# EPFL-VILAB/omnidata

Measured on AMD Instinct MI355X. Metric: images/sec (384x384) DPT-Hybrid surface-normal inference, higher is better.
Workload: dtype bf16; 1 GPU; DPT-Hybrid-384 normal, batch 32/GPU, bf16, 1xMI355X (BASELINE.json configs[1]); batch_per_gpu=32, global_batch=32, parallelism=replicas x1 (no collective in the loop), ranks_seen=1, inflight=1

## Files before the change

### omnidata_amd/csrc/conv1x1.hip

```cpp
#include "gemm_impl.h"

namespace dptx {

constexpr int C1_STG_PITCH = 144;
constexpr int C1_STG_WAVE = 16 * C1_STG_PITCH;
constexpr int C1_WAVES = 4;

template <int KT, int BN>
constexpr size_t conv1x1_smem_bytes() {
  return (size_t)KT * BN * 128 + (size_t)C1_WAVES * KT * 32 * 128 + (size_t)C1_WAVES * C1_STG_WAVE;
}

template <int DT>
__device__ __forceinline__ void c1_unpack8(const u32x4_t v, float* f) {
#pragma unroll
  for (int i = 0; i < 4; ++i) {
    f[2 * i] = T16<DT>::tof((uint16_t)(v[i] & 0xffffu));
    f[2 * i + 1] = T16<DT>::tof((uint16_t)(v[i] >> 16));
  }
}

template <int DT, int KT, int BN, int FORM>
__global__ __launch_bounds__(64 * C1_WAVES, KT <= 2 ? 2 : 1) void conv1x1_stream_kernel(const GemmParams p) {
#if defined(__HIP_DEVICE_COMPILE__)
  constexpr int NSUB = BN / 64;
  constexpr int KS = KT * 4;
  constexpr int W_BYTES = KT * BN * 128;
  constexpr int A_WAVE = KT * 32 * 128;
  extern __shared__ __attribute__((aligned(16))) char smem[];

  const int tid = threadIdx.x;
  const int lane = tid & 63;
  const int wave = __builtin_amdgcn_readfirstlane(tid >> 6);
  const int lr = lane & 31, lh = lane >> 5;

  const int npan = p.N / BN;
  const int x = (int)blockIdx.x & 7, l = (int)blockIdx.x >> 3;
  const int n0 = (l % npan) * BN;
  const int slots = ((int)gridDim.x / npan) * C1_WAVES;
  const int rb_total = (p.M + 31) >> 5;
  int rb = ((l / npan) * 8 + x) * C1_WAVES + wave;

  const int w_bytes = (int)((long long)p.N * p.ldw * 2);
  const __amdgpu_buffer_rsrc_t rsrcA = __builtin_amdgcn_make_buffer_rsrc(const_cast<void*>(p.A), 0, (int)p.a_bytes, 0x00020000);
  const __amdgpu_buffer_rsrc_t rsrcW = __builtin_amdgcn_make_buffer_rsrc(const_cast<void*>(p.W), 0, w_bytes, 0x00020000);

  char* const sw = smem;
  char* const sa = smem + W_BYTES + wave * A_WAVE;
  char* const stg = smem + W_BYTES + C1_WAVES * A_WAVE + wave * C1_STG_WAVE;

  const int kc = lane & 7, r0 = lane >> 3;
  auto issue_a = [&](int rblk) {
#pragma unroll
    for (int i = 0; i < 4; ++i) {
      const int row = r0 + 8 * i;
      const int m = rblk * 32 + row;
      const bool ok = m < p.M;
      const int mm = ok ? m : 0;
      int rem, ox;
      const int img = row_div(mm, p.a_rpi, p.a_rpi_rcp, false, rem);
      const int oy = row_div(rem, p.Wout, p.wout_rcp, false, ox);
      const int iy = oy * p.stride - p.pad_t, ix = ox * p.stride - p.pad_l;
      const bool valid = ok && ((unsigned)iy < (unsigned)p.Hin) && ((unsigned)ix < (unsigned)p.Win);
      const long long e = (long long)img * p.a_img_stride + p.a_off + ((long long)iy * p.Win + ix) * p.a_pix_stride +
                          (kc ^ ((row >> 1) & 7)) * 8;
      const unsigned base = (unsigned)(e * 2);
#pragma unroll
      for (int kt = 0; kt < KT; ++kt) {
        const unsigned vo = valid ? base + kt * 128 : OOB;
        __builtin_amdgcn_raw_ptr_buffer_load_lds(rsrcA, (__attribute__((address_space(3))) void*)(sa + kt * 4096 + i * 1024), 16, vo,
                                                 0, 0, 0);
      }
    }
  };

  if (rb < rb_total) issue_a(rb);
  for (int idx = wave; idx < KT * (BN / 8); idx += C1_WAVES) {
    const int kt = idx / (BN / 8), rg = idx - kt * (BN / 8);
    const int row = rg * 8 + r0;
    const unsigned vo = (unsigned)(((long long)(n0 + row) * p.ldw + kt * 64 + (kc ^ ((row >> 1) & 7)) * 8) * 2);
    __builtin_amdgcn_raw_ptr_buffer_load_lds(rsrcW, (__attribute__((address_space(3))) void*)(sw + kt * (BN * 128) + rg * 1024), 16, vo,
                                             0, 0, 0);
  }
  float bias_c[NSUB][2];
#pragma unroll
  for (int s = 0; s < NSUB; ++s)
#pragma unroll
    for (int j = 0; j < 2; ++j) bias_c[s][j] = FORM == C1_PLAIN && p.bias != nullptr ? p.bias[n0 + s * 64 + j * 32 + lr] : 0.f;
  asm volatile("s_waitcnt vmcnt(0)" ::: "memory");
  __syncthreads();

  const int swz = (lr >> 1) & 7;
  const unsigned sel = (lr & 1) ? 0x03020706u : 0x05040100u;
  const int cn = lane & 7, rr = lane >> 3;

  const bool has_r = FORM == C1_GN && p.R1 != nullptr;
  const bool r_gn = has_r && p.gn_tab_rgn != 0;

  for (; rb < rb_total; rb += slots) {
    const int m0 = rb * 32;
    float ga[NSUB][8], gd[NSUB][8], gra[NSUB][8], grd[NSUB][8];
    u32x4_t rq[NSUB][4];
    auto load_epi = [&](int s) {
      const int img = m0 / p.gn_hw;
      const float* tab = p.gn_tab + (long long)img * 4 * p.N + n0 + s * 64 + cn * 8;
      if (has_r) {
#pragma unroll
        for (int i = 0; i < 4; ++i) {
          const int m = m0 + 16 * (i >> 1) + rr + 8 * (i & 1);
          rq[s][i] = *(const u32x4_t*)((const uint16_t*)p.R1 + (long long)(p.c_row_off + m) * p.ldc + (n0 + s * 64 + cn * 8));
        }
      }
      *(float4*)&ga[s][0] = *(const float4*)(tab);
      *(float4*)&ga[s][4] = *(const float4*)(tab + 4);
      *(float4*)&gd[s][0] = *(const float4*)(tab + p.N);
      *(float4*)&gd[s][4] = *(const float4*)(tab + p.N + 4);
      if (r_gn) {
        *(float4*)&gra[s][0] = *(const float4*)(tab + 2 * p.N);
        *(float4*)&gra[s][4] = *(const float4*)(tab + 2 * p.N + 4);
        *(float4*)&grd[s][0] = *(const float4*)(tab + 3 * p.N);
        *(float4*)&grd[s][4] = *(const float4*)(tab + 3 * p.N + 4);
      }
    };
    if (FORM == C1_GN) load_epi(0);
    u32x4_t af[KS];
#pragma unroll
    for (int ks = 0; ks < KS; ++ks)
      af[ks] = *(const u32x4_t*)(sa + (ks >> 2) * 4096 + lr * 128 + (((2 * (ks & 3) + lh) ^ swz) << 4));
    asm volatile("s_waitcnt lgkmcnt(0)" ::: "memory");
    const bool prefetch = rb + slots < rb_total;
    if (prefetch) issue_a(rb + slots);

#pragma unroll
    for (int s = 0; s < NSUB; ++s) {
      f32x16_t acc[1][2];
#pragma unroll
      for (int j = 0; j < 2; ++j)
#pragma unroll
        for (int r = 0; r < 16; ++r) acc[0][j][r] = 0.f;
#pragma unroll
      for (int kt = 0; kt < KT; ++kt) {
        u32x4_t bf[4][2];
#pragma unroll
        for (int q = 0; q < 4; ++q)
#pragma unroll
          for (int j = 0; j < 2; ++j)
            bf[q][j] = *(const u32x4_t*)(sw + kt * (BN * 128) + (s * 64 + j * 32 + lr) * 128 + (((2 * q + lh) ^ swz) << 4));
        __builtin_amdgcn_sched_barrier(0);
#pragma unroll
        for (int q = 0; q < 4; ++q)
#pragma unroll
          for (int j = 0; j < 2; ++j) acc[0][j] = T16<DT>::mfma32(af[kt * 4 + q], bf[q][j], acc[0][j]);
      }
      if (s == 0) {
        __builtin_amdgcn_sched_barrier(0);
        asm volatile("s_waitcnt vmcnt(0)" ::: "memory");
      }
      if (FORM == C1_STATS || (FORM == C1_PLAIN && p.gn_part != nullptr)) gn_records<1, 2>(p, m0, n0 + s * 64, 0, 0, lr, lh, acc);
      if (FORM == C1_STATS) continue;
      if (FORM == C1_GN && s + 1 < NSUB) load_epi(s + 1);

#pragma unroll
      for (int h = 0; h < 2; ++h) {
        asm volatile("" ::: "memory");
        __builtin_amdgcn_wave_barrier();
#pragma unroll
        for (int j = 0; j < 2; ++j)
#pragma unroll
          for (int t = 0; t < 4; ++t) {
            float v0 = acc[0][j][8 * h + 2 * t] + bias_c[s][j], v1 = acc[0][j][8 * h + 2 * t + 1] + bias_c[s][j];
            if (FORM != C1_GN && p.act == 1) { v0 = fmaxf(v0, 0.f); v1 = fmaxf(v1, 0.f); }
            const uint32_t own = T16<DT>::pack2(v0, v1);
            const uint32_t nb = (uint32_t)__builtin_amdgcn_update_dpp(0, (int)own, 0xB1, 0xf, 0xf, false);
            const uint32_t o = __builtin_amdgcn_perm(nb, own, sel);
            const int rl = ((2 * t) & 3) + (lr & 1) + 8 * (t >> 1) + 4 * lh;
            *(uint32_t*)(stg + rl * C1_STG_PITCH + (j * 32 + (lr & ~1)) * 2) = o;
          }
        asm volatile("" ::: "memory");
        __builtin_amdgcn_wave_barrier();
#pragma unroll
        for (int pp = 0; pp < 2; ++pp) {
          const int rl = rr + 8 * pp;
          u32x4_t d = *(const u32x4_t*)(stg + rl * C1_STG_PITCH + cn * 16);
          const int m = m0 + 16 * h + rl;
          if (FORM == C1_GN) {
            float f[8];
            c1_unpack8<DT>(d, f);
#pragma unroll
            for (int e = 0; e < 8; ++e) f[e] = __builtin_fmaf(f[e], ga[s][e], gd[s][e]);
            if (has_r) {
              float r[8];
              c1_unpack8<DT>(rq[s][2 * h + pp], r);
              if (r_gn) {
#pragma unroll
                for (int e = 0; e < 8; ++e) r[e] = __builtin_fmaf(r[e], gra[s][e], grd[s][e]);
              }
#pragma unroll
              for (int e = 0; e < 8; ++e) f[e] = __fadd_rn(f[e], r[e]);
            }
            if (p.act == 1) {
#pragma unroll
              for (int e = 0; e < 8; ++e) f[e] = fmaxf(f[e], 0.f);
            }
#pragma unroll
            for (int e = 0; e < 4; ++e) d[e] = T16<DT>::pack2(f[2 * e], f[2 * e + 1]);
          }
          if (FORM == C1_GN || m < p.M) *(u32x4_t*)((uint16_t*)p.C + (long long)(p.c_row_off + m) * p.ldc + (n0 + s * 64 + cn * 8)) = d;
        }
      }
    }
  }
#endif
}

bool conv1x1_stream_eligible(int mode, const GemmParams& p) {
  if (mode != MODE_BF16 && mode != MODE_FP16) return false;
  if (p.ksz != 1 || p.pad_t != 0 || p.pad_l != 0 || (p.stride != 1 && p.stride != 2)) return false;
  if (p.K != p.Cin || (p.K != 64 && p.K != 128 && p.K != 256) || p.N % 64 != 0) return false;
  if (p.a_fp32 || p.c_fp32 || p.epi2 || p.a_relu || p.R1 != nullptr || p.R2 != nullptr || p.bias_per_img) return false;
  if (p.c_rpi != 0x7fffffff || p.C8 != nullptr || p.C16 != nullptr || p.out_scale != 0.f) return false;
  if (p.row_stats != nullptr || p.ln_stats != nullptr || (p.act != 0 && p.act != 1)) return false;
  if (p.ldc % 8 != 0 || p.a_pix_stride % 8 != 0 || p.a_off % 8 != 0 || p.a_img_stride % 8 != 0) return false;
  if (p.a_bytes <= 0 || p.a_bytes >= (1ll << 31) || (long long)p.N * p.ldw * 2 >= (1ll << 31) || p.M >= (1 << 23)) return false;
  return true;
}

bool conv1x1_stream_adopted(const GemmParams& p) {
  if (p.stride != 1) return false;
  if (p.K == 64) return p.N == 256 || p.N == 64;
  if (p.K == 128) return p.N == 512;
  if (p.K == 256) return p.N == 64 || p.N == 128 || (p.N == 256 && p.a_rpi >= 48 * 48);
  return false;
}

bool conv1x1_gn_eligible(int mode, const GemmParams& p) {
  if (!conv1x1_stream_eligible(mode, p) || p.stride != 1 || p.bias != nullptr || p.act != 0) return false;
  const int cpg = p.N / 32;
  if (p.a_rpi % 32 != 0 || p.M % p.a_rpi != 0 || p.N > 1024 || (cpg & (cpg - 1)) != 0) return false;
  return p.c_row_off == 0 && p.ldc == p.N;
}

bool conv1x1_gn_adopted(const GemmParams& p) {
  if (p.K == 64) return p.N == 256;
  if (p.K == 128) return p.N == 512;
  return false;
}

template <int DT, int KT, int BN, int FORM>
static hipError_t launch_c1(const GemmParams& p, hipStream_t stream) {
  constexpr size_t smem = conv1x1_smem_bytes<KT, BN>();
  static_assert(smem <= 160 * 1024 && (KT > 2 || 2 * smem <= 160 * 1024), "two blocks per CU at K <= 128");
  const int npan = p.N / BN;
  const int rb_total = (p.M + 31) / 32;
  const int want = (rb_total + C1_WAVES - 1) / C1_WAVES;
  int cap = (KT <= 2 ? 512 : 256) / npan;
  if (cap < 8) cap = 8;
  int groups = want < cap ? want : cap;
  groups = (groups + 7) / 8 * 8;
  auto k = conv1x1_stream_kernel<DT, KT, BN, FORM>;
  set_smem_attr(k, smem);
  hipLaunchKernelGGL(k, dim3(groups * npan), dim3(64 * C1_WAVES), smem, stream, p);
  return hipGetLastError();
}

template <int DT, int FORM>
static hipError_t launch_c1_dt(const GemmParams& p, hipStream_t stream) {
  if (p.K == 64) {
    if constexpr (FORM != C1_GN)
      if (p.N % 256 == 0) return launch_c1<DT, 1, 256, FORM>(p, stream);
    if (p.N % 128 == 0) return launch_c1<DT, 1, 128, FORM>(p, stream);
    return launch_c1<DT, 1, 64, FORM>(p, stream);
  }
  if (p.K == 128) return p.N % 128 == 0 ? launch_c1<DT, 2, 128, FORM>(p, stream) : launch_c1<DT, 2, 64, FORM>(p, stream);
  return p.N % 128 == 0 ? launch_c1<DT, 4, 128, FORM>(p, stream) : launch_c1<DT, 4, 64, FORM>(p, stream);
}

template <int FORM>
static hipError_t launch_c1_form(int mode, const GemmParams& p, hipStream_t stream) {
  return mode == MODE_BF16 ? launch_c1_dt<DT_BF16, FORM>(p, stream) : launch_c1_dt<DT_FP16, FORM>(p, stream);
}

hipError_t launch_conv1x1_stream(int mode, const GemmParams& p0, hipStream_t stream, int form) {
  if (form == C1_PLAIN) {
    if (!conv1x1_stream_eligible(mode, p0) || p0.gn_tab != nullptr) return hipErrorInvalidValue;
    return launch_c1_form<C1_PLAIN>(mode, p0, stream);
  }
  GemmParams p = p0;
  p.trace = nullptr;
  p.a_rpi_rcp = 1.0f / (float)(p.a_rpi > 0 ? p.a_rpi : 1);
  p.wout_rcp = 1.0f / (float)(p.Wout > 0 ? p.Wout : 1);
  GemmParams q = p;
  q.R1 = nullptr; q.act = 0; q.gn_tab = nullptr; q.gn_tab_rgn = 0; q.r1_fp32 = 0;
  if (p.M <= 0 || p.ldw < p.K || p.ldw % 8 != 0 || !conv1x1_gn_eligible(mode, q) || p.r1_fp32) return hipErrorInvalidValue;
  p.gn_hw = p.a_rpi; p.gn_blocks = p.a_rpi / 32; p.gn_cpg = p.N / 32;
  if (form == C1_STATS) {
    if (p.gn_part == nullptr || p.R1 != nullptr || p.act != 0 || p.gn_tab != nullptr) return hipErrorInvalidValue;
    return launch_c1_form<C1_STATS>(mode, p, stream);
  }
  if (form != C1_GN || p.gn_tab == nullptr || p.gn_part != nullptr || p.C == nullptr || p.C == p.R1) return hipErrorInvalidValue;
  return launch_c1_form<C1_GN>(mode, p, stream);
}

}
```

### omnidata_amd/csrc/gemm.hip

```cpp
#include "gemm_impl.h"

namespace dptx {

hipError_t launch_gemm_16(int dt, const GemmParams& p, hipStream_t stream) {
  return dt == DT_BF16 ? launch_dt<DT_BF16, 1>(p, stream) : launch_gemm_fp16(p, stream);
}

void gemm_params_dense(GemmParams& p, int M, int N, int K) {
  p = GemmParams{};
  p.M = M; p.N = N; p.K = K; p.ldw = K;
  p.a_rpi = M > 0 ? M : 1; p.Wout = p.a_rpi; p.Hin = 1; p.Win = p.a_rpi; p.Cin = K; p.a_pix_stride = K;
  p.a_img_stride = 0; p.a_off = 0; p.ksz = 1; p.stride = 1; p.pad_t = 0; p.pad_l = 0;
  p.c_rpi = 0x7fffffff; p.c_img_rows = 0; p.c_row_off = 0; p.ldc = N;
  p.a_bytes = (long long)M * K * 2;
}

void gemm_params_conv(GemmParams& p, int B, int Hin, int Win, int Cin, int Cout, int ksz, int stride, int pad_t, int pad_l,
                      int Hout, int Wout, int a_elem_bytes) {
  p = GemmParams{};
  p.M = B * Hout * Wout; p.N = Cout; p.K = ksz * ksz * Cin; p.ldw = p.K;
  p.a_rpi = Hout * Wout; p.Wout = Wout; p.Hin = Hin; p.Win = Win; p.Cin = Cin; p.a_pix_stride = Cin;
  p.a_img_stride = (long long)Hin * Win * Cin; p.a_off = 0; p.ksz = ksz; p.stride = stride; p.pad_t = pad_t; p.pad_l = pad_l;
  p.c_rpi = 0x7fffffff; p.c_img_rows = 0; p.c_row_off = 0; p.ldc = Cout;
  p.a_bytes = (long long)B * Hin * Win * Cin * a_elem_bytes;
  p.k_tap_fast = (ksz == 3 && Cin >= 512) ? 1 : 0;
}

static thread_local long long* g_trace = nullptr;
void gemm_set_trace(long long* dev_buf) { g_trace = dev_buf; }
static thread_local int g_debug_flags = 0;
void gemm_set_debug_flags(int flags) { g_debug_flags = flags; }
int gemm_debug_flags() { return g_debug_flags; }
static thread_local float g_cu_share = 1.0f;
void gemm_set_cu_share(float share) { g_cu_share = share > 0.f && share <= 1.f ? share : 1.0f; }

hipError_t launch_gemm(int mode, const GemmParams& p0, hipStream_t stream) {
  GemmParams p = p0;
  p.trace = g_trace;
  p.debug_flags = g_debug_flags;
  if (p.cu_share <= 0.f) p.cu_share = g_cu_share;
  p.a_rpi_rcp = 1.0f / (float)(p.a_rpi > 0 ? p.a_rpi : 1);
  p.wout_rcp = 1.0f / (float)(p.Wout > 0 ? p.Wout : 1);
  if (p.gn_part != nullptr && (p.gn_hw % 32 != 0 || p.N % 32 != 0 || p.gn_cpg != p.N / 32 || p.gn_cpg < 2 || p.gn_cpg > 32 ||
                               (p.gn_cpg & (p.gn_cpg - 1)) != 0 || p.bias != nullptr || p.act != 0))
    return hipErrorInvalidValue;
  if (p.row_stats != nullptr && (p.N % 128 != 0 || p.stats_nblk != 8 || p.N / 128 > 8)) return hipErrorInvalidValue;
  if (p.ln_stats != nullptr && (p.R1 != nullptr || p.R2 != nullptr || p.bias_per_img || p.ln_colsum == nullptr || (p.ln_nblk != 6 && p.ln_nblk != 8) ||
                                p.c_rpi != 0x7fffffff || p.gn_part != nullptr))
    return hipErrorInvalidValue;
  if (mode == MODE_FP8) {
    if (p.K % 128 != 0 || p.Cin % 128 != 0 || p.M <= 0 || p.N % 32 != 0 || p.ldw < p.K || p.ldw % 16 != 0 || p.gn_part != nullptr)
      return hipErrorInvalidValue;
    return launch_gemm_fp8(p, stream);
  }
  if (p.K % BK != 0 || p.Cin % BK != 0 || p.M <= 0 || p.N % 32 != 0 || p.ldw < p.K || p.ldw % 8 != 0) return hipErrorInvalidValue;
  if (!(p.debug_flags & 8) && conv1x1_stream_eligible(mode, p) && ((p.debug_flags & 16) || conv1x1_stream_adopted(p)))
    return launch_conv1x1_stream(mode, p, stream);
  if (mode == MODE_BF16) return p.epi2 ? hipErrorInvalidValue : launch_gemm_16(DT_BF16, p, stream);
  if (mode == MODE_FP16) return p.epi2 ? launch_gemm_fp16e(p, stream) : launch_gemm_16(DT_FP16, p, stream);
  if (mode == MODE_BF16X3) return launch_gemm_x3(DT_BF16, p, stream);
  if (mode == MODE_FP16X3) return p.a_hi_only ? launch_gemm_x2(p, stream) : launch_gemm_x3(DT_FP16, p, stream);
  return hipErrorInvalidValue;
}

}
```

### omnidata_amd/csrc/norm.hip

```cpp
#include "common.h"
#include "kernels.h"

namespace dptx {

template <int DT, int PL, int VPL>
__global__ __launch_bounds__(256) void layernorm_kernel(const float* __restrict__ x, const float* __restrict__ gamma,
                                                        const float* __restrict__ beta, uint16_t* __restrict__ y,
                                                        int M, int C, float eps, long long plane) {
  const int lane = threadIdx.x & 63;
  const int row = blockIdx.x * 4 + (threadIdx.x >> 6);
  if (row >= M) return;
  const float* xr = x + (long long)row * C;
  float4 v[VPL];
  float s = 0.f;
#pragma unroll
  for (int j = 0; j < VPL; ++j) {
    v[j] = *(const float4*)(xr + (j * 64 + lane) * 4);
    s += (v[j].x + v[j].y) + (v[j].z + v[j].w);
  }
  const float mean = wave_sum(s) / (float)C;
  float q = 0.f;
#pragma unroll
  for (int j = 0; j < VPL; ++j) {
    const float a = v[j].x - mean, b = v[j].y - mean, c = v[j].z - mean, d = v[j].w - mean;
    q += (a * a + b * b) + (c * c + d * d);
  }
  const float rstd = rsqrtf(wave_sum(q) / (float)C + eps);
  uint16_t* yr = y + (long long)row * C;
#pragma unroll
  for (int j = 0; j < VPL; ++j) {
    const int c0 = (j * 64 + lane) * 4;
    const float4 g = *(const float4*)(gamma + c0), bb = *(const float4*)(beta + c0);
    const float o0 = (v[j].x - mean) * rstd * g.x + bb.x, o1 = (v[j].y - mean) * rstd * g.y + bb.y;
    const float o2 = (v[j].z - mean) * rstd * g.z + bb.z, o3 = (v[j].w - mean) * rstd * g.w + bb.w;
    uint2 w;
    w.x = T16<DT>::pack2(o0, o1);
    w.y = T16<DT>::pack2(o2, o3);
    *(uint2*)(yr + c0) = w;
    if (PL == 2) {
      uint2 l;
      l.x = T16<DT>::pack2(o0 - T16<DT>::tof((uint16_t)(w.x & 0xffffu)), o1 - T16<DT>::tof((uint16_t)(w.x >> 16)));
      l.y = T16<DT>::pack2(o2 - T16<DT>::tof((uint16_t)(w.y & 0xffffu)), o3 - T16<DT>::tof((uint16_t)(w.y >> 16)));
      *(uint2*)(yr + plane + c0) = l;
    }
  }
}

hipError_t launch_layernorm(int mode, const float* x, const float* gamma, const float* beta, void* y, int M, int C,
                            float eps, Planes pl, hipStream_t stream) {
  if (C != 768 && C != 1024) return hipErrorInvalidValue;
  dim3 grid((M + 3) / 4);
  if (C == 768) {
    DPTX_DISPATCH_MODE(mode, hipLaunchKernelGGL((layernorm_kernel<DT, PL, 3>), grid, dim3(256), 0, stream, x, gamma, beta,
                                                (uint16_t*)y, M, C, eps, pl.act));
  } else {
    DPTX_DISPATCH_MODE(mode, hipLaunchKernelGGL((layernorm_kernel<DT, PL, 4>), grid, dim3(256), 0, stream, x, gamma, beta,
                                                (uint16_t*)y, M, C, eps, pl.act));
  }
  return hipGetLastError();
}

constexpr int GN_G = 32;

static inline int gn_pix(int C) {
  const int pix = 16384 / C;
  return pix < 16 ? 16 : (pix > 256 ? 256 : pix);
}
int gn_chunks(int HW, int C) {
  const int pix = gn_pix(C);
  return (HW + pix - 1) / pix;
}

template <int DT, int PL>
__global__ __launch_bounds__(256) void gn_stats_kernel(const uint16_t* __restrict__ X, float* __restrict__ partial,
                                                       int HW, int C, int pix, long long plane) {
  __shared__ float red[256 * 8];
  const int tid = threadIdx.x;
  const int cvec = C >> 3;
  const int cpg = C >> 5;
  const int spv = cpg >= 8 ? 1 : 8 / cpg;
  const int v = tid % cvec, p0 = tid / cvec, pstep = 256 / cvec;
  const int b = blockIdx.y, chunk = blockIdx.x;
  const int pbeg = chunk * pix;
  const int pend = min(pbeg + pix, HW);
  float s[4] = {0.f, 0.f, 0.f, 0.f}, q[4] = {0.f, 0.f, 0.f, 0.f};
  const uint16_t* base = X + ((long long)b * HW) * C + v * 8;
  for (int p = pbeg + p0; p < pend; p += pstep) {
    float f[8];
    load8f<DT, PL>(base + (long long)p * C, plane, f);
    if (spv == 1) {
#pragma unroll
      for (int e = 0; e < 8; ++e) { s[0] += f[e]; q[0] += f[e] * f[e]; }
    } else if (spv == 2) {
#pragma unroll
      for (int e = 0; e < 4; ++e) { s[0] += f[e]; q[0] += f[e] * f[e]; s[1] += f[4 + e]; q[1] += f[4 + e] * f[4 + e]; }
    } else {
#pragma unroll
      for (int e = 0; e < 4; ++e) { s[e] += f[2 * e] + f[2 * e + 1]; q[e] += f[2 * e] * f[2 * e] + f[2 * e + 1] * f[2 * e + 1]; }
    }
  }
#pragma unroll
  for (int e = 0; e < 4; ++e) { red[tid * 8 + 2 * e] = s[e]; red[tid * 8 + 2 * e + 1] = q[e]; }
  __syncthreads();
  if (tid < GN_G) {
    const int g = tid;
    int v0, v1, slot;
    if (spv == 1) { v0 = g * (cpg >> 3); v1 = v0 + (cpg >> 3); slot = 0; }
    else { v0 = g / spv; v1 = v0 + 1; slot = g % spv; }
    float ss = 0.f, qq = 0.f;
    for (int pp = 0; pp < pstep; ++pp)
      for (int vv = v0; vv < v1; ++vv) {
        const int t = pp * cvec + vv;
        ss += red[t * 8 + 2 * slot];
        qq += red[t * 8 + 2 * slot + 1];
      }
    float* out = partial + (((long long)b * gridDim.x + chunk) * GN_G + g) * 2;
    out[0] = ss;
    out[1] = qq;
  }
}

hipError_t launch_gn_stats(int mode, const void* X, float* partial, int B, int HW, int C, Planes pl, hipStream_t stream) {
  if (C % 64 != 0 || C > 1024 || (256 % (C / 8)) != 0) return hipErrorInvalidValue;
  dim3 grid(gn_chunks(HW, C), B);
  DPTX_DISPATCH_MODE(mode, hipLaunchKernelGGL((gn_stats_kernel<DT, PL>), grid, dim3(256), 0, stream, (const uint16_t*)X, partial,
                                              HW, C, gn_pix(C), pl.act));
  return hipGetLastError();
}

__device__ __forceinline__ void gn_affine_to_lds(const float* __restrict__ partial, int nchunks, int b,
                                                 const float* __restrict__ gamma, const float* __restrict__ beta, int C,
                                                 int HW, float eps, float* sa, float* sd, float* smr) {
  __shared__ double sred[8][GN_G][2];
  const int tid = threadIdx.x;
  const int cpg = C >> 5;
  {
    const int g = tid & (GN_G - 1), slice = tid >> 5;
    double ss = 0.0, qq = 0.0;
    const float2* pp = (const float2*)partial + (long long)b * nchunks * GN_G + g;
    for (int c = slice; c < nchunks; c += 8) {
      const float2 v = pp[(long long)c * GN_G];
      ss += (double)v.x;
      qq += (double)v.y;
    }
    sred[slice][g][0] = ss;
    sred[slice][g][1] = qq;
  }
  __syncthreads();
  if (tid < GN_G) {
    double ss = 0.0, qq = 0.0;
#pragma unroll
    for (int sl = 0; sl < 8; ++sl) { ss += sred[sl][tid][0]; qq += sred[sl][tid][1]; }
    const double n = (double)HW * (double)cpg;
    const double mean = ss / n;
    double var = qq / n - mean * mean;
    if (var < 0.0) var = 0.0;
    smr[2 * tid] = (float)mean;
    smr[2 * tid + 1] = (float)(1.0 / sqrt(var + (double)eps));
  }
  __syncthreads();
  for (int c = tid; c < C; c += blockDim.x) {
    const int g = c / cpg;
    const float a = __fmul_rn(smr[2 * g + 1], gamma[c]);
    sa[c] = a;
    sd[c] = __builtin_fmaf(-a, smr[2 * g], beta[c]);
  }
  __syncthreads();
}

template <int DT, int PL>
__global__ __launch_bounds__(256) void gn_apply_kernel(const GnParams p, int pix, int nrec, long long plane) {
  __shared__ float sa[1024], sd[1024], ra[1024], rd[1024], smr[64];
  const int b = blockIdx.y;
  gn_affine_to_lds(p.partial, nrec, b, p.gamma, p.beta, p.C, p.HW, p.eps, sa, sd, smr);
  const bool r_gn = (p.R != nullptr) && (p.r_gamma != nullptr);
  if (r_gn) gn_affine_to_lds(p.r_partial, nrec, b, p.r_gamma, p.r_beta, p.C, p.HW, p.eps, ra, rd, smr);
  const int cvec = p.C >> 3;
  const int pbeg = blockIdx.x * pix;
  const int pend = min(pbeg + pix, p.HW);
  const long long img = (long long)b * p.HW * p.C;
  const uint16_t* X = (const uint16_t*)p.X + img;
  const uint16_t* R = p.R ? (const uint16_t*)p.R + img : nullptr;
  uint16_t* Y = (uint16_t*)p.Y + img;
  const int total = (pend - pbeg) * cvec;
  for (int i = threadIdx.x; i < total; i += 256) {
    const int pi = i / cvec, v = i - pi * cvec;
    const long long off = (long long)(pbeg + pi) * p.C + v * 8;
    float f[8];
    load8f<DT, PL>(X + off, plane, f);
#pragma unroll
    for (int e = 0; e < 8; ++e) f[e] = __builtin_fmaf(f[e], sa[v * 8 + e], sd[v * 8 + e]);
    if (R != nullptr) {
      float r[8];
      load8f<DT, PL>(R + off, plane, r);
      if (r_gn) {
#pragma unroll
        for (int e = 0; e < 8; ++e) r[e] = __builtin_fmaf(r[e], ra[v * 8 + e], rd[v * 8 + e]);
      }
#pragma unroll
      for (int e = 0; e < 8; ++e) f[e] = __fadd_rn(f[e], r[e]);
    }
    if (p.relu) {
#pragma unroll
      for (int e = 0; e < 8; ++e) f[e] = fmaxf(f[e], 0.f);
    }
    store8f<DT, PL>(Y + off, plane, f);
  }
}

hipError_t launch_gn_apply(int mode, const GnParams& p, Planes pl, hipStream_t stream) {
  if (p.C % 64 != 0 || p.C > 1024) return hipErrorInvalidValue;
  const int nch = gn_chunks(p.HW, p.C);
  const int nrec = p.nrec > 0 ? p.nrec : nch;
  int nb = nch;
  if (p.nrec > 0) {
    int want = 1024 / (p.B > 0 ? p.B : 1);
    want = want < 4 ? 4 : want;
    nb = nch < want ? nch : want;
  }
  const int pix = (p.HW + nb - 1) / nb;
  dim3 grid((p.HW + pix - 1) / pix, p.B);
  DPTX_DISPATCH_MODE(mode, hipLaunchKernelGGL((gn_apply_kernel<DT, PL>), grid, dim3(256), 0, stream, p, pix, nrec, pl.act));
  return hipGetLastError();
}

__global__ __launch_bounds__(256) void gn_finalize_kernel(const float* __restrict__ partial, const float* __restrict__ gamma,
                                                          const float* __restrict__ beta, const float* __restrict__ r_partial,
                                                          const float* __restrict__ r_gamma, const float* __restrict__ r_beta,
                                                          float* __restrict__ tab, int nrec, int C, int HW, float eps) {
  __shared__ float smr[64];
  const int b = blockIdx.x, t = blockIdx.y;
  float* const ta = tab + ((long long)b * 4 + 2 * t) * C;
  gn_affine_to_lds(t ? r_partial : partial, nrec, b, t ? r_gamma : gamma, t ? r_beta : beta, C, HW, eps, ta, ta + C, smr);
}

hipError_t launch_gn_finalize(const float* partial, const float* gamma, const float* beta, const float* r_partial,
                              const float* r_gamma, const float* r_beta, float* tab, int B, int HW, int C, int nrec, float eps,
                              hipStream_t stream) {
  if (C % 64 != 0 || C > 1024 || B <= 0 || nrec <= 0 || partial == nullptr || gamma == nullptr || beta == nullptr || tab == nullptr)
    return hipErrorInvalidValue;
  if (r_partial != nullptr && (r_gamma == nullptr || r_beta == nullptr)) return hipErrorInvalidValue;
  hipLaunchKernelGGL(gn_finalize_kernel, dim3(B, r_partial != nullptr ? 2 : 1), dim3(256), 0, stream, partial, gamma, beta,
                     r_partial, r_gamma, r_beta, tab, nrec, C, HW, eps);
  return hipGetLastError();
}

template <int DT, int PL>
__global__ __launch_bounds__(256) void gn_relu_maxpool_kernel(const uint16_t* __restrict__ X, uint16_t* __restrict__ Y,
                                                              const float* __restrict__ gamma, const float* __restrict__ beta,
                                                              const float* __restrict__ partial, int nchunks, int H, int W,
                                                              int C, float eps, long long plane) {
  __shared__ float sa[1024], sd[1024], smr[64];
  const int b = blockIdx.y;
  gn_affine_to_lds(partial, nchunks, b, gamma, beta, C, H * W, eps, sa, sd, smr);
  const int Ho = (H + 1) / 2, Wo = (W + 1) / 2;
  const int cvec = C >> 3;
  const int total = Ho * Wo * cvec;
  const uint16_t* Xi = X + (long long)b * H * W * C;
  uint16_t* Yo = Y + (long long)b * Ho * Wo * C;
  for (int i = blockIdx.x * 256 + threadIdx.x; i < total; i += gridDim.x * 256) {
    const int v = i % cvec, po = i / cvec;
    const int oy = po / Wo, ox = po - oy * Wo;
    float m[8];
#pragma unroll
    for (int e = 0; e < 8; ++e) m[e] = 0.f;
#pragma unroll
    for (int dy = 0; dy < 3; ++dy) {
      const int iy = 2 * oy + dy;
      if (iy >= H) continue;
#pragma unroll
      for (int dx = 0; dx < 3; ++dx) {
        const int ix = 2 * ox + dx;
        if (ix >= W) continue;
        float f[8];
        load8f<DT, PL>(Xi + ((long long)iy * W + ix) * C + v * 8, plane, f);
#pragma unroll
        for (int e = 0; e < 8; ++e) m[e] = fmaxf(m[e], f[e] * sa[v * 8 + e] + sd[v * 8 + e]);
      }
    }
    store8f<DT, PL>(Yo + (long long)po * C + v * 8, plane, m);
  }
}

hipError_t launch_gn_relu_maxpool(int mode, const void* X, void* Y, const float* gamma, const float* beta,
                                  const float* partial, int B, int H, int W, int C, float eps, Planes pl, hipStream_t stream) {
  if ((H & 1) || (W & 1) || C % 64 != 0 || C > 1024) return hipErrorInvalidValue;
  const int Ho = (H + 1) / 2, Wo = (W + 1) / 2;
  const int total = Ho * Wo * (C / 8);
  dim3 grid(min((total + 255) / 256, 64), B);
  const int nch = gn_chunks(H * W, C);
  DPTX_DISPATCH_MODE(mode, hipLaunchKernelGGL((gn_relu_maxpool_kernel<DT, PL>), grid, dim3(256), 0, stream, (const uint16_t*)X,
                                              (uint16_t*)Y, gamma, beta, partial, nch, H, W, C, eps, pl.act));
  return hipGetLastError();
}

}
```

Baseline: 2747 images/s.

## Add half-K 8-wave conv1x1 stream path for K=256 and batch GN partial loads

Adds a K=256 variant of the streaming 1x1-conv kernel. It uses 8 waves per block and stages only half of the A tile at a time, loading the second K half while MFMAs run on the first. The smaller per-wave LDS footprint allows more waves, and the kernel is adopted by default for selected K=256 layer shapes. Separately, the GroupNorm affine reduction now issues 12 partial loads before accumulating, to raise memory-level parallelism; the old serial chain is kept behind a debug flag. The cost is more accumulator registers live at once and extra waits in the half-K pipeline.

Result: no change. 2773 images/s (median of 6 runs) (+0.9%).

```diff
diff --git a/omnidata_amd/csrc/conv1x1.hip b/omnidata_amd/csrc/conv1x1.hip
--- a/omnidata_amd/csrc/conv1x1.hip
+++ b/omnidata_amd/csrc/conv1x1.hip
@@ -6,9 +6,9 @@
 constexpr int C1_STG_WAVE = 16 * C1_STG_PITCH;
 constexpr int C1_WAVES = 4;
 
-template <int KT, int BN>
+template <int KT, int BN, int WAVES = C1_WAVES, int HK = 0>
 constexpr size_t conv1x1_smem_bytes() {
-  return (size_t)KT * BN * 128 + (size_t)C1_WAVES * KT * 32 * 128 + (size_t)C1_WAVES * C1_STG_WAVE;
+  return (size_t)KT * BN * 128 + (size_t)WAVES * (HK ? 2 : KT) * 32 * 128 + (size_t)WAVES * C1_STG_WAVE;
 }
 
 template <int DT>
@@ -20,13 +20,15 @@
   }
 }
 
-template <int DT, int KT, int BN, int FORM>
-__global__ __launch_bounds__(64 * C1_WAVES, KT <= 2 ? 2 : 1) void conv1x1_stream_kernel(const GemmParams p) {
+template <int DT, int KT, int BN, int FORM, int WAVES = C1_WAVES, int HK = 0>
+__global__ __launch_bounds__(64 * WAVES, KT <= 2 ? 2 : 1) void conv1x1_stream_kernel(const GemmParams p) {
 #if defined(__HIP_DEVICE_COMPILE__)
   constexpr int NSUB = BN / 64;
   constexpr int KS = KT * 4;
   constexpr int W_BYTES = KT * BN * 128;
-  constexpr int A_WAVE = KT * 32 * 128;
+  constexpr int KTB = HK ? 2 : KT;
+  constexpr int A_WAVE = KTB * 32 * 128;
+  static_assert(!HK || (KT == 4 && BN == 128), "the half-K form: K = 256, two 64-column passes");
   extern __shared__ __attribute__((aligned(16))) char smem[];
 
   const int tid = threadIdx.x;
@@ -37,9 +39,9 @@
   const int npan = p.N / BN;
   const int x = (int)blockIdx.x & 7, l = (int)blockIdx.x >> 3;
   const int n0 = (l % npan) * BN;
-  const int slots = ((int)gridDim.x / npan) * C1_WAVES;
+  const int slots = ((int)gridDim.x / npan) * WAVES;
   const int rb_total = (p.M + 31) >> 5;
-  int rb = ((l / npan) * 8 + x) * C1_WAVES + wave;
+  int rb = ((l / npan) * 8 + x) * WAVES + wave;
 
   const int w_bytes = (int)((long long)p.N * p.ldw * 2);
   const __amdgpu_buffer_rsrc_t rsrcA = __builtin_amdgcn_make_buffer_rsrc(const_cast<void*>(p.A), 0, (int)p.a_bytes, 0x00020000);
@@ -47,10 +49,10 @@
 
   char* const sw = smem;
   char* const sa = smem + W_BYTES + wave * A_WAVE;
-  char* const stg = smem + W_BYTES + C1_WAVES * A_WAVE + wave * C1_STG_WAVE;
+  char* const stg = smem + W_BYTES + WAVES * A_WAVE + wave * C1_STG_WAVE;
 
   const int kc = lane & 7, r0 = lane >> 3;
-  auto issue_a = [&](int rblk) {
+  auto issue_a = [&](int rblk, int kt0 = 0) {
 #pragma unroll
     for (int i = 0; i < 4; ++i) {
       const int row = r0 + 8 * i;
@@ -66,8 +68,8 @@
                           (kc ^ ((row >> 1) & 7)) * 8;
       const unsigned base = (unsigned)(e * 2);
 #pragma unroll
-      for (int kt = 0; kt < KT; ++kt) {
-        const unsigned vo = valid ? base + kt * 128 : OOB;
+      for (int kt = 0; kt < KTB; ++kt) {
+        const unsigned vo = valid ? base + (kt0 + kt) * 128 : OOB;
         __builtin_amdgcn_raw_ptr_buffer_load_lds(rsrcA, (__attribute__((address_space(3))) void*)(sa + kt * 4096 + i * 1024), 16, vo,
                                                  0, 0, 0);
       }
@@ -75,7 +77,7 @@
   };
 
   if (rb < rb_total) issue_a(rb);
-  for (int idx = wave; idx < KT * (BN / 8); idx += C1_WAVES) {
+  for (int idx = wave; idx < KT * (BN / 8); idx += WAVES) {
     const int kt = idx / (BN / 8), rg = idx - kt * (BN / 8);
     const int row = rg * 8 + r0;
     const unsigned vo = (unsigned)(((long long)(n0 + row) * p.ldw + kt * 64 + (kc ^ ((row >> 1) & 7)) * 8) * 2);
@@ -99,66 +101,100 @@
 
   for (; rb < rb_total; rb += slots) {
     const int m0 = rb * 32;
-    float ga[NSUB][8], gd[NSUB][8], gra[NSUB][8], grd[NSUB][8];
-    u32x4_t rq[NSUB][4];
+    constexpr int EB = HK ? 1 : NSUB;
+    float ga[EB][8], gd[EB][8], gra[EB][8], grd[EB][8];
+    u32x4_t rq[EB][4];
     auto load_epi = [&](int s) {
+      const int eb = HK ? 0 : s;
       const int img = m0 / p.gn_hw;
       const float* tab = p.gn_tab + (long long)img * 4 * p.N + n0 + s * 64 + cn * 8;
       if (has_r) {
 #pragma unroll
         for (int i = 0; i < 4; ++i) {
           const int m = m0 + 16 * (i >> 1) + rr + 8 * (i & 1);
-          rq[s][i] = *(const u32x4_t*)((const uint16_t*)p.R1 + (long long)(p.c_row_off + m) * p.ldc + (n0 + s * 64 + cn * 8));
+          rq[eb][i] = *(const u32x4_t*)((const uint16_t*)p.R1 + (long long)(p.c_row_off + m) * p.ldc + (n0 + s * 64 + cn * 8));
         }
       }
-      *(float4*)&ga[s][0] = *(const float4*)(tab);
-      *(float4*)&ga[s][4] = *(const float4*)(tab + 4);
-      *(float4*)&gd[s][0] = *(const float4*)(tab + p.N);
-      *(float4*)&gd[s][4] = *(const float4*)(tab + p.N + 4);
+      *(float4*)&ga[eb][0] = *(const float4*)(tab);
+      *(float4*)&ga[eb][4] = *(const float4*)(tab + 4);
+      *(float4*)&gd[eb][0] = *(const float4*)(tab + p.N);
+      *(float4*)&gd[eb][4] = *(const float4*)(tab + p.N + 4);
       if (r_gn) {
-        *(float4*)&gra[s][0] = *(const float4*)(tab + 2 * p.N);
-        *(float4*)&gra[s][4] = *(const float4*)(tab + 2 * p.N + 4);
-        *(float4*)&grd[s][0] = *(const float4*)(tab + 3 * p.N);
-        *(float4*)&grd[s][4] = *(const float4*)(tab + 3 * p.N + 4);
+        *(float4*)&gra[eb][0] = *(const float4*)(tab + 2 * p.N);
+        *(float4*)&gra[eb][4] = *(const float4*)(tab + 2 * p.N + 4);
+        *(float4*)&grd[eb][0] = *(const float4*)(tab + 3 * p.N);
+        *(float4*)&grd[eb][4] = *(const float4*)(tab + 3 * p.N + 4);
       }
     };
     if (FORM == C1_GN) load_epi(0);
-    u32x4_t af[KS];
-#pragma unroll
-    for (int ks = 0; ks < KS; ++ks)
-      af[ks] = *(const u32x4_t*)(sa + (ks >> 2) * 4096 + lr * 128 + (((2 * (ks & 3) + lh) ^ swz) << 4));
-    asm volatile("s_waitcnt lgkmcnt(0)" ::: "memory");
+    u32x4_t af[KTB * 4];
+    auto read_a = [&]() {
+#pragma unroll
+      for (int ks = 0; ks < KTB * 4; ++ks)
+        af[ks] = *(const u32x4_t*)(sa + (ks >> 2) * 4096 + lr * 128 + (((2 * (ks & 3) + lh) ^ swz) << 4));
+      asm volatile("s_waitcnt lgkmcnt(0)" ::: "memory");
+    };
+    auto mfma_pass = [&](int s, int kt0, f32x16_t (&acc)[1][2]) {
+#pragma unroll
+      for (int kt = 0; kt < KTB; ++kt) {
+        u32x4_t bf[4][2];
+#pragma unroll
+        for (int q = 0; q < 4; ++q)
+#pragma unroll
+          for (int j = 0; j < 2; ++j)
+            bf[q][j] = *(const u32x4_t*)(sw + (kt0 + kt) * (BN * 128) + (s * 64 + j * 32 + lr) * 128 + (((2 * q + lh) ^ swz) << 4));
+        __builtin_amdgcn_sched_barrier(0);
+#pragma unroll
+        for (int q = 0; q < 4; ++q)
+#pragma unroll
+          for (int j = 0; j < 2; ++j) acc[0][j] = T16<DT>::mfma32(af[kt * 4 + q], bf[q][j], acc[0][j]);
+      }
+    };
     const bool prefetch = rb + slots < rb_total;
-    if (prefetch) issue_a(rb + slots);
+    f32x16_t accs[HK ? NSUB : 1][1][2];
+    if constexpr (HK) {
+#pragma unroll
+      for (int s = 0; s < NSUB; ++s)
+#pragma unroll
+        for (int j = 0; j < 2; ++j)
+#pragma unroll
+          for (int r = 0; r < 16; ++r) accs[s][0][j][r] = 0.f;
+      read_a();
+      issue_a(rb, 2);
+#pragma unroll
+      for (int s = 0; s < NSUB; ++s) mfma_pass(s, 0, accs[s]);
+      __builtin_amdgcn_sched_barrier(0);
+      asm volatile("s_waitcnt vmcnt(0)" ::: "memory");
+      read_a();
+      if (prefetch) issue_a(rb + slots, 0);
+#pragma unroll
+      for (int s = 0; s < NSUB; ++s) mfma_pass(s, 2, accs[s]);
+      __builtin_amdgcn_sched_barrier(0);
+      asm volatile("s_waitcnt vmcnt(0)" ::: "memory");
+    } else {
+      read_a();
+      if (prefetch) issue_a(rb + slots);
+    }
 
 #pragma unroll
     for (int s = 0; s < NSUB; ++s) {
-      f32x16_t acc[1][2];
-#pragma unroll
-      for (int j = 0; j < 2; ++j)
-#pragma unroll
-        for (int r = 0; r < 16; ++r) acc[0][j][r] = 0.f;
-#pragma unroll
-      for (int kt = 0; kt < KT; ++kt) {
-        u32x4_t bf[4][2];
-#pragma unroll
-        for (int q = 0; q < 4; ++q)
-#pragma unroll
-          for (int j = 0; j < 2; ++j)
-            bf[q][j] = *(const u32x4_t*)(sw + kt * (BN * 128) + (s * 64 + j * 32 + lr) * 128 + (((2 * q + lh) ^ swz) << 4));
-        __builtin_amdgcn_sched_barrier(0);
-#pragma unroll
-        for (int q = 0; q < 4; ++q)
-#pragma unroll
-          for (int j = 0; j < 2; ++j) acc[0][j] = T16<DT>::mfma32(af[kt * 4 + q], bf[q][j], acc[0][j]);
-      }
-      if (s == 0) {
-        __builtin_amdgcn_sched_barrier(0);
-        asm volatile("s_waitcnt vmcnt(0)" ::: "memory");
+      f32x16_t(&acc)[1][2] = accs[HK ? s : 0];
+      const int eb = HK ? 0 : s;
+      if constexpr (!HK) {
+#pragma unroll
+        for (int j = 0; j < 2; ++j)
+#pragma unroll
+          for (int r = 0; r < 16; ++r) acc[0][j][r] = 0.f;
+        mfma_pass(s, 0, acc);
+        if (s == 0) {
+          __builtin_amdgcn_sched_barrier(0);
+          asm volatile("s_waitcnt vmcnt(0)" ::: "memory");
+        }
       }
       if (FORM == C1_STATS || (FORM == C1_PLAIN && p.gn_part != nullptr)) gn_records<1, 2>(p, m0, n0 + s * 64, 0, 0, lr, lh, acc);
       if (FORM == C1_STATS) continue;
-      if (FORM == C1_GN && s + 1 < NSUB) load_epi(s + 1);
+      if (FORM == C1_GN && s > 0 && HK) load_epi(s);
+      if (FORM == C1_GN && s + 1 < NSUB && !HK) load_epi(s + 1);
 
 #pragma unroll
       for (int h = 0; h < 2; ++h) {
@@ -187,13 +223,13 @@
             float f[8];
             c1_unpack8<DT>(d, f);
 #pragma unroll
-            for (int e = 0; e < 8; ++e) f[e] = __builtin_fmaf(f[e], ga[s][e], gd[s][e]);
+            for (int e = 0; e < 8; ++e) f[e] = __builtin_fmaf(f[e], ga[eb][e], gd[eb][e]);
             if (has_r) {
               float r[8];
-              c1_unpack8<DT>(rq[s][2 * h + pp], r);
+              c1_unpack8<DT>(rq[eb][2 * h + pp], r);
               if (r_gn) {
 #pragma unroll
-                for (int e = 0; e < 8; ++e) r[e] = __builtin_fmaf(r[e], gra[s][e], grd[s][e]);
+                for (int e = 0; e < 8; ++e) r[e] = __builtin_fmaf(r[e], gra[eb][e], grd[eb][e]);
               }
 #pragma unroll
               for (int e = 0; e < 8; ++e) f[e] = __fadd_rn(f[e], r[e]);
@@ -225,7 +261,14 @@
   return true;
 }
 
+static bool conv1x1_k256_adopted(const GemmParams& p) {
+  if (p.K != 256 || p.N % 128 != 0) return false;
+  if (p.stride != 1) return p.N == 512;
+  return p.N == 1024 || p.N == 128 || (p.N == 256 && p.a_rpi == 48 * 48);
+}
+
 bool conv1x1_stream_adopted(const GemmParams& p) {
+  if (conv1x1_k256_adopted(p)) return true;
   if (p.stride != 1) return false;
   if (p.K == 64) return p.N == 256 || p.N == 64;
   if (p.K == 128) return p.N == 512;
@@ -246,20 +289,20 @@
   return false;
 }
 
-template <int DT, int KT, int BN, int FORM>
+template <int DT, int KT, int BN, int FORM, int WAVES = C1_WAVES, int HK = 0>
 static hipError_t launch_c1(const GemmParams& p, hipStream_t stream) {
-  constexpr size_t smem = conv1x1_smem_bytes<KT, BN>();
-  static_assert(smem <= 160 * 1024 && (KT > 2 || 2 * smem <= 160 * 1024), "two blocks per CU at K <= 128");
+  constexpr size_t smem = conv1x1_smem_bytes<KT, BN, WAVES, HK>();
+  static_assert(smem <= 160 * 1024 && (KT > 2 || 2 * smem <= 160 * 1024), "two blocks per CU at K <= 128, one at K = 256");
   const int npan = p.N / BN;
   const int rb_total = (p.M + 31) / 32;
-  const int want = (rb_total + C1_WAVES - 1) / C1_WAVES;
+  const int want = (rb_total + WAVES - 1) / WAVES;
   int cap = (KT <= 2 ? 512 : 256) / npan;
   if (cap < 8) cap = 8;
   int groups = want < cap ? want : cap;
   groups = (groups + 7) / 8 * 8;
-  auto k = conv1x1_stream_kernel<DT, KT, BN, FORM>;
+  auto k = conv1x1_stream_kernel<DT, KT, BN, FORM, WAVES, HK>;
   set_smem_attr(k, smem);
-  hipLaunchKernelGGL(k, dim3(groups * npan), dim3(64 * C1_WAVES), smem, stream, p);
+  hipLaunchKernelGGL(k, dim3(groups * npan), dim3(64 * WAVES), smem, stream, p);
   return hipGetLastError();
 }
 
@@ -272,6 +315,8 @@
     return launch_c1<DT, 1, 64, FORM>(p, stream);
   }
   if (p.K == 128) return p.N % 128 == 0 ? launch_c1<DT, 2, 128, FORM>(p, stream) : launch_c1<DT, 2, 64, FORM>(p, stream);
+  const int flags = gemm_debug_flags();
+  if (p.N % 128 == 0 && ((flags & 1024) || (!(flags & 16) && conv1x1_k256_adopted(p)))) return launch_c1<DT, 4, 128, FORM, 8, 1>(p, stream);
   return p.N % 128 == 0 ? launch_c1<DT, 4, 128, FORM>(p, stream) : launch_c1<DT, 4, 64, FORM>(p, stream);
 }
 
diff --git a/omnidata_amd/csrc/gemm.hip b/omnidata_amd/csrc/gemm.hip
--- a/omnidata_amd/csrc/gemm.hip
+++ b/omnidata_amd/csrc/gemm.hip
@@ -54,7 +54,8 @@
     return launch_gemm_fp8(p, stream);
   }
   if (p.K % BK != 0 || p.Cin % BK != 0 || p.M <= 0 || p.N % 32 != 0 || p.ldw < p.K || p.ldw % 8 != 0) return hipErrorInvalidValue;
-  if (!(p.debug_flags & 8) && conv1x1_stream_eligible(mode, p) && ((p.debug_flags & 16) || conv1x1_stream_adopted(p)))
+  if (!(p.debug_flags & 8) && conv1x1_stream_eligible(mode, p) &&
+      ((p.debug_flags & 16) || ((p.debug_flags & 1024) && p.K == 256 && p.N % 128 == 0) || conv1x1_stream_adopted(p)))
     return launch_conv1x1_stream(mode, p, stream);
   if (mode == MODE_BF16) return p.epi2 ? hipErrorInvalidValue : launch_gemm_16(DT_BF16, p, stream);
   if (mode == MODE_FP16) return p.epi2 ? launch_gemm_fp16e(p, stream) : launch_gemm_16(DT_FP16, p, stream);
diff --git a/omnidata_amd/csrc/norm.hip b/omnidata_amd/csrc/norm.hip
--- a/omnidata_amd/csrc/norm.hip
+++ b/omnidata_amd/csrc/norm.hip
@@ -128,9 +128,10 @@
   return hipGetLastError();
 }
 
+constexpr int GN_LB = 12;
 __device__ __forceinline__ void gn_affine_to_lds(const float* __restrict__ partial, int nchunks, int b,
                                                  const float* __restrict__ gamma, const float* __restrict__ beta, int C,
-                                                 int HW, float eps, float* sa, float* sd, float* smr) {
+                                                 int HW, float eps, float* sa, float* sd, float* smr, int chain) {
   __shared__ double sred[8][GN_G][2];
   const int tid = threadIdx.x;
   const int cpg = C >> 5;
@@ -138,10 +139,29 @@
     const int g = tid & (GN_G - 1), slice = tid >> 5;
     double ss = 0.0, qq = 0.0;
     const float2* pp = (const float2*)partial + (long long)b * nchunks * GN_G + g;
-    for (int c = slice; c < nchunks; c += 8) {
-      const float2 v = pp[(long long)c * GN_G];
-      ss += (double)v.x;
-      qq += (double)v.y;
+    if (chain) {
+      for (int c = slice; c < nchunks; c += 8) {
+        const float2 v = pp[(long long)c * GN_G];
+        ss += (double)v.x;
+        qq += (double)v.y;
+      }
+    } else {
+      int c = slice;
+      for (; c + 8 * (GN_LB - 1) < nchunks; c += 8 * GN_LB) {
+        float2 v[GN_LB];
+#pragma unroll
+        for (int j = 0; j < GN_LB; ++j) v[j] = pp[(long long)(c + 8 * j) * GN_G];
+#pragma unroll
+        for (int j = 0; j < GN_LB; ++j) { ss += (double)v[j].x; qq += (double)v[j].y; }
+      }
+      if (c < nchunks) {
+        float2 v[GN_LB - 1];
+#pragma unroll
+        for (int j = 0; j < GN_LB - 1; ++j) v[j] = pp[(long long)min(c + 8 * j, nchunks - 1) * GN_G];
+#pragma unroll
+        for (int j = 0; j < GN_LB - 1; ++j)
+          if (c + 8 * j < nchunks) { ss += (double)v[j].x; qq += (double)v[j].y; }
+      }
     }
     sred[slice][g][0] = ss;
     sred[slice][g][1] = qq;
@@ -169,12 +189,12 @@
 }
 
 template <int DT, int PL>
-__global__ __launch_bounds__(256) void gn_apply_kernel(const GnParams p, int pix, int nrec, long long plane) {
+__global__ __launch_bounds__(256) void gn_apply_kernel(const GnParams p, int pix, int nrec, long long plane, int chain) {
   __shared__ float sa[1024], sd[1024], ra[1024], rd[1024], smr[64];
   const int b = blockIdx.y;
-  gn_affine_to_lds(p.partial, nrec, b, p.gamma, p.beta, p.C, p.HW, p.eps, sa, sd, smr);
+  gn_affine_to_lds(p.partial, nrec, b, p.gamma, p.beta, p.C, p.HW, p.eps, sa, sd, smr, chain);
   const bool r_gn = (p.R != nullptr) && (p.r_gamma != nullptr);
-  if (r_gn) gn_affine_to_lds(p.r_partial, nrec, b, p.r_gamma, p.r_beta, p.C, p.HW, p.eps, ra, rd, smr);
+  if (r_gn) gn_affine_to_lds(p.r_partial, nrec, b, p.r_gamma, p.r_beta, p.C, p.HW, p.eps, ra, rd, smr, chain);
   const int cvec = p.C >> 3;
   const int pbeg = blockIdx.x * pix;
   const int pend = min(pbeg + pix, p.HW);
@@ -220,18 +240,19 @@
   }
   const int pix = (p.HW + nb - 1) / nb;
   dim3 grid((p.HW + pix - 1) / pix, p.B);
-  DPTX_DISPATCH_MODE(mode, hipLaunchKernelGGL((gn_apply_kernel<DT, PL>), grid, dim3(256), 0, stream, p, pix, nrec, pl.act));
+  const int chain = gemm_debug_flags() & 512;
+  DPTX_DISPATCH_MODE(mode, hipLaunchKernelGGL((gn_apply_kernel<DT, PL>), grid, dim3(256), 0, stream, p, pix, nrec, pl.act, chain));
   return hipGetLastError();
 }
 
 __global__ __launch_bounds__(256) void gn_finalize_kernel(const float* __restrict__ partial, const float* __restrict__ gamma,
                                                           const float* __restrict__ beta, const float* __restrict__ r_partial,
                                                           const float* __restrict__ r_gamma, const float* __restrict__ r_beta,
-                                                          float* __restrict__ tab, int nrec, int C, int HW, float eps) {
+                                                          float* __restrict__ tab, int nrec, int C, int HW, float eps, int chain) {
   __shared__ float smr[64];
   const int b = blockIdx.x, t = blockIdx.y;
   float* const ta = tab + ((long long)b * 4 + 2 * t) * C;
-  gn_affine_to_lds(t ? r_partial : partial, nrec, b, t ? r_gamma : gamma, t ? r_beta : beta, C, HW, eps, ta, ta + C, smr);
+  gn_affine_to_lds(t ? r_partial : partial, nrec, b, t ? r_gamma : gamma, t ? r_beta : beta, C, HW, eps, ta, ta + C, smr, chain);
 }
 
 hipError_t launch_gn_finalize(const float* partial, const float* gamma, const float* beta, const float* r_partial,
@@ -241,7 +262,7 @@
     return hipErrorInvalidValue;
   if (r_partial != nullptr && (r_gamma == nullptr || r_beta == nullptr)) return hipErrorInvalidValue;
   hipLaunchKernelGGL(gn_finalize_kernel, dim3(B, r_partial != nullptr ? 2 : 1), dim3(256), 0, stream, partial, gamma, beta,
-                     r_partial, r_gamma, r_beta, tab, nrec, C, HW, eps);
+                     r_partial, r_gamma, r_beta, tab, nrec, C, HW, eps, gemm_debug_flags() & 512);
   return hipGetLastError();
 }
 
@@ -249,10 +270,10 @@
 __global__ __launch_bounds__(256) void gn_relu_maxpool_kernel(const uint16_t* __restrict__ X, uint16_t* __restrict__ Y,
                                                               const float* __restrict__ gamma, const float* __restrict__ beta,
                                                               const float* __restrict__ partial, int nchunks, int H, int W,
-                                                              int C, float eps, long long plane) {
+                                                              int C, float eps, long long plane, int chain) {
   __shared__ float sa[1024], sd[1024], smr[64];
   const int b = blockIdx.y;
-  gn_affine_to_lds(partial, nchunks, b, gamma, beta, C, H * W, eps, sa, sd, smr);
+  gn_affine_to_lds(partial, nchunks, b, gamma, beta, C, H * W, eps, sa, sd, smr, chain);
   const int Ho = (H + 1) / 2, Wo = (W + 1) / 2;
   const int cvec = C >> 3;
   const int total = Ho * Wo * cvec;
@@ -289,9 +310,10 @@
   const int total = Ho * Wo * (C / 8);
   dim3 grid(min((total + 255) / 256, 64), B);
   const int nch = gn_chunks(H * W, C);
+  const int chain = gemm_debug_flags() & 512;
   DPTX_DISPATCH_MODE(mode, hipLaunchKernelGGL((gn_relu_maxpool_kernel<DT, PL>), grid, dim3(256), 0, stream, (const uint16_t*)X,
-                                              (uint16_t*)Y, gamma, beta, partial, nch, H, W, C, eps, pl.act));
-  return hipGetLastError();
-}
-
-}
+                                              (uint16_t*)Y, gamma, beta, partial, nch, H, W, C, eps, pl.act, chain));
+  return hipGetLastError();
+}
+
+}
```
